# yuang-chen/of-spmm

Hardware: AMD Instinct MI355X
Metric: SpMM effective GFLOP/s + achieved HBM GB/s vs roofline, 1/2/4/8 MI355X (higher is better)
Workload: dtype f32; 1 GPU; products: CSR 2449029x2449029, 123718280 nnz x dense N=128; m=2449029, k=2449029, nnz=123718280, n=128, index=int32, parallelism=single GPU

## Files before the change

of-spmm_amd/csrc/ofx_internal.h:

```cpp
#ifndef OFX_INTERNAL_H_
#define OFX_INTERNAL_H_

#include <stdarg.h>
#include <stdint.h>
#include <stdio.h>

#include "ofx_spmm.h"

namespace ofx {
int fail(int code, const char* fmt, ...) __attribute__((format(printf, 2, 3)));
void clear_error();

int guard_exception(const char* fn);
template <typename F>
inline int guarded(const char* fn, F&& body) noexcept {
  try {
    return body();
  } catch (...) {
    return guard_exception(fn);
  }
}

unsigned* device_error_words();
int take_device_error(const char* where);
int64_t debug_knob(int knob, int64_t dflt);

const char* versioned_struct_problem(const void* p, uint32_t min_size);
int read_options(const ofx_spmm_options* in, ofx_spmm_options* out, const char* fn);
}

#define OFX_READ_OPTIONS(opts, fn)                                                 \
  ofx_spmm_options ofx_opts_copy_;                                                 \
  do {                                                                             \
    if (const int ofx_ro_ = ::ofx::read_options((opts), &ofx_opts_copy_, (fn))) return ofx_ro_; \
    (opts) = &ofx_opts_copy_;                                                      \
  } while (0)

#define OFX_TAKE_DEVICE_ERROR(where)                                    \
  do {                                                                  \
    if (const int ofx_de_ = ::ofx::take_device_error(where)) return ofx_de_; \
  } while (0)

#define OFX_HIP_CHECK(expr)                                                                 \
  do {                                                                                      \
    hipError_t ofx_e_ = (expr);                                                             \
    if (ofx_e_ != hipSuccess) {                                                             \
      (void)hipGetLastError();       \
      return ::ofx::fail(OFX_EDEVICE, "%s failed: %s (%s:%d)", #expr,                       \
                         hipGetErrorString(ofx_e_), __FILE__, __LINE__);                    \
    }                                                                                       \
  } while (0)

#define OFX_REQUIRE(cond, code, ...)              \
  do {                                            \
    if (!(cond)) return ::ofx::fail(code, __VA_ARGS__); \
  } while (0)

#endif
```

of-spmm_amd/csrc/spmm_common.h:

```cpp
#ifndef OFX_SPMM_COMMON_H_
#define OFX_SPMM_COMMON_H_

#include <stdint.h>
#include <string.h>

#include "ofx_spmm.h"

#if defined(__HIPCC__) || defined(__HIP__)
#include <hip/hip_runtime.h>
#define OFX_HD __host__ __device__ __forceinline__
#else
#define OFX_HD static inline
#endif

namespace ofx {

struct bf16 {
  uint16_t x;
};
struct f16 {
  uint16_t x;
};

OFX_HD float bits_to_f32(uint32_t u) { return __builtin_bit_cast(float, u); }
OFX_HD uint32_t f32_to_bits(float f) { return __builtin_bit_cast(uint32_t, f); }

OFX_HD float bf16_to_f32(uint16_t h) { return bits_to_f32(uint32_t(h) << 16); }
OFX_HD uint16_t f32_to_bf16(float f) {
#if defined(__HIP_DEVICE_COMPILE__)
  return __builtin_bit_cast(uint16_t, (__bf16)f);
#else
  const uint32_t u = f32_to_bits(f);
  if ((u & 0x7fffffffu) > 0x7f800000u) return uint16_t((u >> 16) | 0x40u);
  return uint16_t((u + 0x7fffu + ((u >> 16) & 1u)) >> 16);
#endif
}
OFX_HD float f16_to_f32(uint16_t h) { return float(__builtin_bit_cast(_Float16, h)); }
OFX_HD uint16_t f32_to_f16(float f) { return __builtin_bit_cast(uint16_t, _Float16(f)); }

OFX_HD float round_bf16(float f) {
#if defined(__HIP_DEVICE_COMPILE__)
  return (float)(__bf16)f;
#else
  const uint32_t u = f32_to_bits(f);
  if ((u & 0x7fffffffu) > 0x7f800000u) return bits_to_f32((u & 0xffff0000u) | 0x400000u);
  return bits_to_f32((u + 0x7fffu + ((u >> 16) & 1u)) & 0xffff0000u);
#endif
}

template <typename T>
struct Num;
template <>
struct Num<float> {
  using acc = float;
  OFX_HD static float load(float v) { return v; }
  OFX_HD static float store(float a) { return a; }
  OFX_HD static float mul(float v, float b) { return v * b; }
};
template <>
struct Num<double> {
  using acc = double;
  OFX_HD static double load(double v) { return v; }
  OFX_HD static double store(double a) { return a; }
  OFX_HD static double mul(double v, double b) { return v * b; }
};
template <>
struct Num<bf16> {
  using acc = float;
  OFX_HD static float load(bf16 v) { return bf16_to_f32(v.x); }
  OFX_HD static bf16 store(float a) { return bf16{f32_to_bf16(a)}; }
  OFX_HD static float mul(float v, float b) { return round_bf16(v * b); }
};
template <>
struct Num<f16> {
  using acc = float;
  OFX_HD static float load(f16 v) { return f16_to_f32(v.x); }
  OFX_HD static f16 store(float a) { return f16{f32_to_f16(a)}; }
  OFX_HD static float mul(float v, float b) { return float(_Float16(v * b)); }
};

template <typename T>
OFX_HD T epilogue(typename Num<T>::acc acc, const T* bias, int64_t c, int act) {
  T y = Num<T>::store(acc);
  if (bias) y = Num<T>::store(Num<T>::load(y) + Num<T>::load(bias[c]));
  if (act == OFX_ACT_RELU && Num<T>::load(y) <= typename Num<T>::acc(0))
    y = Num<T>::store(typename Num<T>::acc(0));
  return y;
}

template <typename T>
OFX_HD T poison_value() {
  return Num<T>::store(typename Num<T>::acc(__builtin_nan("")));
}

OFX_HD int dtype_size(int dt) {
  switch (dt) {
    case OFX_DT_FLOAT: return 4;
    case OFX_DT_DOUBLE: return 8;
    case OFX_DT_INT32: return 4;
    case OFX_DT_INT64: return 8;
    case OFX_DT_FLOAT16: return 2;
    case OFX_DT_BFLOAT16: return 2;
    default: return 0;
  }
}
OFX_HD bool is_index_dtype(int dt) { return dt == OFX_DT_INT32 || dt == OFX_DT_INT64; }
OFX_HD bool is_value_dtype(int dt) {
  return dt == OFX_DT_FLOAT || dt == OFX_DT_DOUBLE || dt == OFX_DT_FLOAT16 ||
         dt == OFX_DT_BFLOAT16;
}

OFX_HD int64_t default_split(int64_t n) {
  int64_t t = n > 0 ? (int64_t)65536 / n : 512;
  if (t < 128) t = 128;
  if (t > 512) t = 512;
  int64_t p = 128;
  while (p * 2 <= t) p *= 2;
  return p;
}

struct Schedule {
  int64_t split;
  int64_t chunk;
  int64_t heavy;
  int32_t variant;
  int32_t planned;
  int32_t force_bin;
};

static inline Schedule resolve_schedule(int64_t n, const ofx_spmm_options* o) {
  Schedule s;
  s.variant = o ? o->variant : 0;
  s.planned = o ? o->planned : 0;
  s.force_bin = 0;
  const int64_t h = o ? o->heavy_threshold : 0;
  s.heavy = h > 0 ? h : (h < 0 ? INT64_MAX : 0);
  if (o && o->ordered) {
    s.split = INT64_MAX;
    s.chunk = INT64_MAX;
    return s;
  }
  s.split = (o && o->split_threshold > 0) ? o->split_threshold : default_split(n);
  s.chunk = (o && o->chunk > 0) ? o->chunk : s.split;
  if (s.chunk > s.split) s.chunk = s.split;
  return s;
}

OFX_HD int64_t auto_heavy(int64_t nrows, int64_t nnz) {
  const int64_t mean = nrows > 0 ? (nnz + nrows - 1) / nrows : 1;
  return 5 * mean < 16 ? 16 : 5 * mean;
}

OFX_HD int64_t num_chunks(int64_t len, int64_t chunk) { return len / chunk; }

OFX_HD uint64_t splitmix64(uint64_t x) {
  x += 0x9e3779b97f4a7c15ull;
  x = (x ^ (x >> 30)) * 0xbf58476d1ce4e5b9ull;
  x = (x ^ (x >> 27)) * 0x94d049bb133111ebull;
  return x ^ (x >> 31);
}
OFX_HD uint64_t hash2(uint64_t seed, uint64_t i) { return splitmix64(splitmix64(seed) ^ i); }
OFX_HD float u_pm1(uint64_t h) { return float((int64_t)(h >> 40) - (1 << 23)) * (1.0f / (1 << 23)); }
OFX_HD float exact_val(uint64_t h) {
  const float t[4] = {-2.f, -1.f, 1.f, 2.f};
  return t[(h >> 33) & 3];
}
OFX_HD float exact_dense(uint64_t h) { return float((int)((h >> 33) % 17) - 8); }

}

#endif
```

of-spmm_amd/csrc/spmm_csr_impl.h:

```cpp
#ifndef OFX_SPMM_CSR_IMPL_H_
#define OFX_SPMM_CSR_IMPL_H_
#pragma clang fp contract(off)

#include <hip/hip_runtime.h>

#include <algorithm>
#include <climits>
#include <cstdio>
#include <cstring>
#include <type_traits>

#include "ofx_internal.h"
#include "spmm_common.h"
#include "spmm_plan.h"
#include "spmm_launch.h"
#include "dbg_bounds.h"

namespace ofx {
namespace {


using plan::WorkList;
using plan::WsLayout;
using plan::launch_plan;
// ... 741 lines not shown
          PA x[QR];
#pragma unroll
          for (int q = 0; q < QR; ++q)
            if (i + q < cnt) x[q] = *reinterpret_cast<const PA*>(buf + (i + q) * W + gl * VEC);
#pragma unroll
          for (int q = 0; q < QR; ++q)
            if (i + q < cnt)
#pragma unroll
              for (int e = 0; e < VEC; ++e) acc[e] = acc[e] + x[q].v[e];
        }
      }
    }
  };
  span_load(0, rc, rv);
  span_store(0, rc, rv);
  __syncthreads();
  span_load(1, rc, rv);
  static_assert(D == 4, "small form: the load ring below is written out for D = 4");
  P b0[UW], b1[UW], b2[UW], b3[UW];
  issue(0, b0);
  issue(1, b1);
  issue(2, b2);
  issue(3, b3);
  static_assert(S == 2 * D, "small form: a span is two turns of the ring");
  int64_t k0 = 0;
  for (; k0 + S <= nb; k0 += S) {
    step(k0 + 0, b0, false);
    step(k0 + 1, b1, false);
    step(k0 + 2, b2, false);
    step(k0 + 3, b3, false);
    step(k0 + 4, b0, true);
    step(k0 + 5, b1, false);
    step(k0 + 6, b2, false);
    step(k0 + 7, b3, false);
  }
  if (k0 + 0 < nb) step(k0 + 0, b0, false);
  if (k0 + 1 < nb) step(k0 + 1, b1, false);
  if (k0 + 2 < nb) step(k0 + 2, b2, false);
  if (k0 + 3 < nb) step(k0 + 3, b3, false);
  if (k0 + 4 < nb) step(k0 + 4, b0, false);
  if (k0 + 5 < nb) step(k0 + 5, b1, false);
  if (k0 + 6 < nb) step(k0 + 6, b2, false);
  if (kpc > 0) {
#pragma unroll
    for (int e = 0; e < VEC; ++e) acc[e] = total[e] + acc[e];
  }
  __syncthreads();
}

template <typename T, typename I, typename K>
__global__ void __launch_bounds__(64 * K::WPB)
    spmm_small_kernel(const I* __restrict__ rp, const I* __restrict__ col,
                      const T* __restrict__ val, const I* __restrict__ vperm,
                      const T* __restrict__ B, int64_t ldb, int64_t kb, T* __restrict__ C,
                      int64_t ldc, int64_t row_begin, int64_t nrows, int64_t n, int64_t split,
                      int64_t chunk,
                      int64_t light, const T* __restrict__ bias, int act) {
  using SF = SmallForm<T, I, K>;
  using A = typename Num<T>::acc;
  constexpr int VEC = K::VEC, LPR = K::LPR, W = SF::W, RPB = SF::RPB;
  __shared__ __attribute__((aligned(16))) SmallLds<T, I, K> lds;
  __shared__ int heavy_rows[RPB];
  __shared__ int nheavy;
  const int lane = threadIdx.x & 63;
  const int wave = threadIdx.x >> 6;
  const int gl = lane & (LPR - 1);
  const int gbase = lane & ~(LPR - 1);
  const int q = LPR == 64 ? 0 : lane / LPR;
  const int gb = wave * SF::G + q;
  const int64_t row0 = (int64_t)blockIdx.x * RPB;
  if (threadIdx.x == 0) nheavy = 0;
  __syncthreads();
  const int64_t lr = row0 + gb;
  if (lr < nrows) {
    const int64_t rs = (int64_t)OFX_LD(rp + (row_begin + lr));
    const int64_t re = (int64_t)OFX_LD(rp + (row_begin + lr + 1));
    const int64_t len = re - rs;
    if (len > light || len > split) {
      if (gl == 0) heavy_rows[atomicAdd(&nheavy, 1)] = gb;
    } else {
      for (int64_t c0 = 0; c0 < n; c0 += W) {
        const int64_t cc = c0 + (int64_t)gl * VEC;
        const bool active = cc < n;
        A acc[VEC];
#pragma unroll
        for (int e = 0; e < VEC; ++e) acc[e] = A(0);
        accumulate<T, I, K>(col, val, vperm, brows<T, K::BUF>(B, c0, cc, active, ldb, kb), rs, re, gl, gbase,
                            active, acc);
        if (active) store_row<T, VEC, K::NT>(C + lr * ldc + cc, acc, bias ? bias + cc : nullptr, act);
      }
    }
  }
  __syncthreads();
  const int nh = nheavy;
  const bool chain = wave == 0 && q == 0;
  for (int h = 0; h < nh; ++h) {
    const int64_t hr = row0 + heavy_rows[h];
    const int64_t rs = (int64_t)OFX_LD(rp + (row_begin + hr));
    const int64_t re = (int64_t)OFX_LD(rp + (row_begin + hr + 1));
    const bool split_row = re - rs > split;
    const int64_t nc = split_row ? num_chunks(re - rs, chunk) : 1;
    const bool one_pass = split_row && chunk % SF::NB == 0;
    for (int64_t c0 = 0; c0 < n; c0 += W) {
      const int64_t cc = c0 + (int64_t)gl * VEC;
      const bool active = cc < n;
      const BRows<T, K::BUF> br = brows<T, K::BUF>(B, c0, cc, active, ldb, kb);
      A total[VEC], acc[VEC];
#pragma unroll
      for (int e = 0; e < VEC; ++e) total[e] = A(0);
      if (one_pass) {
#pragma unroll
        for (int e = 0; e < VEC; ++e) acc[e] = A(0);
        block_accumulate<T, I, K>(col, val, vperm, br, rs, re, gb, gl, chain, lds, acc,
                                  chunk / SF::NB, nc);
        if (chain && active) store_row<T, VEC, K::NT>(C + hr * ldc + cc, acc, bias ? bias + cc : nullptr, act);
        continue;
      }
      for (int64_t ci = 0; ci < nc; ++ci) {
        int64_t j0 = rs, j1 = re;
        if (split_row) {
          j0 = rs + ci * chunk;
          j1 = (re - j0 - chunk < chunk) ? re : j0 + chunk;
        }
#pragma unroll
        for (int e = 0; e < VEC; ++e) acc[e] = A(0);
        block_accumulate<T, I, K>(col, val, vperm, br, j0, j1, gb, gl, chain, lds, acc);
        if (split_row) {
#pragma unroll
          for (int e = 0; e < VEC; ++e) total[e] = total[e] + acc[e];
        }
      }
      if (chain && active)
        store_row<T, VEC, K::NT>(C + hr * ldc + cc, split_row ? total : acc,
                                 bias ? bias + cc : nullptr, act);
    }
  }
}

#ifdef OFX_AB_WPE
#define OFX_MAIN_WPE __attribute__((amdgpu_waves_per_eu(OFX_AB_WPE)))
#else
#define OFX_MAIN_WPE
#endif
template <typename T>
__device__ __attribute__((noinline)) void poison_output(T* __restrict__ C, int64_t ldc,
                                                        int64_t nrows, int64_t n) {
  const T p = poison_value<T>();
  const int64_t total = nrows * n;
  const int64_t stride = (int64_t)gridDim.x * blockDim.x;
  for (int64_t e = (int64_t)blockIdx.x * blockDim.x + threadIdx.x; e < total; e += stride)
    C[(e / n) * ldc + e % n] = p;
}

template <typename T, typename I, typename K>
__global__ void __launch_bounds__(64 * K::WPB) OFX_MAIN_WPE
    spmm_main_kernel(const I* __restrict__ rp, const I* __restrict__ col,
                     const T* __restrict__ val, const I* __restrict__ vperm,
                     const T* __restrict__ B, int64_t ldb, int64_t kb,
                     T* __restrict__ C, int64_t ldc, int64_t row_begin, int64_t nrows, int64_t n,
                     int64_t split, int64_t chunk, int64_t heavy,
                     const unsigned long long* __restrict__ counters,
                     const int64_t* __restrict__ items, const int64_t* __restrict__ order,
                     typename Num<T>::acc* __restrict__ part, const T* __restrict__ bias,
                     int act, int64_t wave_blocks, int64_t block_base,
                     unsigned* __restrict__ arrive, unsigned* err) {
  using A = typename Num<T>::acc;
  constexpr int VEC = K::VEC, LPR = K::LPR, kWaves = K::WPB;
  const int64_t bid = block_base + (int64_t)blockIdx.x;
  if (counters != nullptr && !plan::plan_valid(counters)) {
    if (bid == 0 && threadIdx.x == 0) plan::raise_device_error(err, plan::kErrPlanInvalid);
    poison_output<T>(C, ldc, nrows, n);
    return;
  }
  constexpr int GPW = 64 / LPR;
  const int lane = threadIdx.x & 63;
  const int wave = __builtin_amdgcn_readfirstlane(threadIdx.x >> 6);
  const int gl = lane & (LPR - 1);
  const int gbase = lane & ~(LPR - 1);
  const int gsub = LPR == 64 ? 0 : lane / LPR;
  if constexpr (K::WH && LPR < 64) {
    using KW = WaveMap<K>;
    constexpr int WV = KW::VEC, WL = KW::LPR;
    if (bid < wave_blocks) {
      const int wgl = lane & (WL - 1);
      const int64_t nchunks = (int64_t)OFX_LD(counters + 0);
      const int64_t nheavy = (int64_t)OFX_LD(counters + 3) - (int64_t)OFX_LD(counters + 2);
      for (int64_t w = bid * kWaves + wave; w < nchunks + nheavy; w += wave_blocks * kWaves) {
        int64_t wr, wc = -1;
        if (w < nchunks) {
          wr = OFX_LD(items + (2 * w + 0));
          wc = OFX_LD(items + (2 * w + 1));
        } else {
          wr = plan::order_row(order, nrows, nheavy, w - nchunks);
        }
        wr = uniform64(wr);
        wc = uniform64(wc);
        const int64_t rs = (int64_t)OFX_LD(rp + (row_begin + wr));
        const int64_t re = (int64_t)OFX_LD(rp + (row_begin + wr + 1));
        int64_t j0 = rs, j1 = re;
        if (wc >= 0) {
          j0 = rs + wc * chunk;
          j1 = (re - j0 - chunk < chunk) ? re : j0 + chunk;
        }
        for (int64_t c0 = 0; c0 < n; c0 += (int64_t)WL * WV) {
          int64_t cc = c0 + (int64_t)wgl * WV;
          const bool active = cc < n;
          if constexpr (K::SH && WV > 1) {
            if (active && cc + WV > n) cc = n - WV;
          }
          A acc[WV];
#pragma unroll
          for (int e = 0; e < WV; ++e) acc[e] = A(0);
          if constexpr (K::XL) {
            __shared__ A xl_lds[K::WPB][KW::XL_FLOATS];
            accumulate_wave_xl<T, I, KW>(col, val, vperm, brows<T, K::BUF>(B, c0, cc, active, ldb, kb),
                                         j0, j1, lane, wgl, xl_lds[wave], acc);
          } else {
            accumulate_wave<T, I, KW>(col, val, vperm, brows<T, K::BUF>(B, c0, cc, active, ldb, kb),
                                      j0, j1, lane, wgl, acc);
          }
          if (active && lane < WL) {
            if (wc >= 0)
              store_partial<A, WV, K::LR>(part + w * n + cc, acc);
            else
              store_row<T, WV, K::NT>(C + wr * ldc + cc, acc, bias ? bias + cc : nullptr, act);
          }
        }
        if constexpr (K::LR) {
          if (wc >= 0)
            hub_tail<T, WV, WL, K::SH && (WV > 1)>(arrive, w - wc, num_chunks(re - rs, chunk), part, C, ldc,
                                       wr, n, wgl, lane < WL, 0, bias, act);
        }
      }
      return;
    }
  }
  if constexpr (K::BI) {
    if (bid < wave_blocks) {
      __shared__ __attribute__((aligned(16))) SmallLds<T, I, K> lds;
      constexpr int W = SmallForm<T, I, K>::W;
      const int64_t w = bid;
      const int64_t nchunks = (int64_t)OFX_LD(counters + 0);
      const int64_t nheavy = (int64_t)OFX_LD(counters + 3) - (int64_t)OFX_LD(counters + 2);
      if (w >= nchunks + nheavy) return;
      int64_t wr, wc = -1;
      if (w < nchunks) {
        wr = OFX_LD(items + (2 * w + 0));
        wc = OFX_LD(items + (2 * w + 1));
      } else {
        wr = plan::order_row(order, nrows, nheavy, w - nchunks);
      }
      wr = uniform64(wr);
      wc = uniform64(wc);
      const int64_t rs = (int64_t)OFX_LD(rp + (row_begin + wr));
      const int64_t re = (int64_t)OFX_LD(rp + (row_begin + wr + 1));
      int64_t j0 = rs, j1 = re;
      if (wc >= 0) {
        j0 = rs + wc * chunk;
        j1 = (re - j0 - chunk < chunk) ? re : j0 + chunk;
      }
      const int gb = wave * GPW + gsub;
      const bool chain = wave == 0 && gsub == 0;
      for (int64_t c0 = 0; c0 < n; c0 += W) {
        const int64_t cc = c0 + (int64_t)gl * VEC;
        const bool active = cc < n;
        A acc[VEC];
#pragma unroll
        for (int e = 0; e < VEC; ++e) acc[e] = A(0);
        block_accumulate<T, I, K>(col, val, vperm, brows<T, K::BUF>(B, c0, cc, active, ldb, kb), j0, j1, gb, gl,
                                  chain, lds, acc);
        if (chain && active) {
          if (wc >= 0)
            store_partial<A, VEC, K::LR>(part + w * n + cc, acc);
          else
            store_row<T, VEC, K::NT>(C + wr * ldc + cc, acc, bias ? bias + cc : nullptr, act);
        }
      }
      if constexpr (K::LR) {
        if (wc >= 0 && chain)
          hub_tail<T, VEC, LPR, K::SH>(arrive, w - wc, num_chunks(re - rs, chunk), part, C, ldc, wr,
                                       n, gl, true, gbase, bias, act);
      }
      return;
    }
  }
  int64_t g = ((bid - ((K::WH || K::BI) ? wave_blocks : 0)) * kWaves + wave) * GPW +
              gsub;
  if constexpr ((K::WH && LPR < 64) || K::BI) {
    if (order != nullptr)
      g += (int64_t)OFX_LD(counters + 0) + (int64_t)OFX_LD(counters + 3) -
           (int64_t)OFX_LD(counters + 2);
  }
  constexpr int64_t kIdxExcluded = 16;
#if defined(OFX_LIGHT_ORDER)
  constexpr bool kIdx = false;
#else
  constexpr bool kIdx = true;
#endif
  int64_t lr, c = -1;
  bool by_index = false;
  if (order == nullptr) {
    if (g >= nrows) return;
    lr = g;
  } else {
    const int64_t nchunks = (int64_t)OFX_LD(counters + 0);
    const int64_t nhubs = (int64_t)OFX_LD(counters + 1);
    const int64_t nheavy = (int64_t)OFX_LD(counters + 3) - (int64_t)OFX_LD(counters + 2);
#if defined(OFX_LIGHT_INDEX)
    const bool idx = true;
#else
    const bool idx = kIdx && (nhubs + nheavy) * kIdxExcluded <= nrows;
#endif
    if (g < nchunks) {
      lr = OFX_LD(items + (2 * g + 0));
      c = OFX_LD(items + (2 * g + 1));
    } else if (g < nchunks + nheavy || !idx) {
      const int64_t q = g - nchunks;
      if (q >= nrows - nhubs) return;
      lr = plan::order_row(order, nrows, nheavy, q);
    } else {
      lr = g - nchunks - nheavy;
      if (lr >= nrows) return;
      by_index = true;
    }
  }
  if constexpr (LPR == 64) {
    lr = uniform64(lr);
    c = uniform64(c);
  }
  const int64_t rs = (int64_t)OFX_LD(rp + (row_begin + lr));
  const int64_t re = (int64_t)OFX_LD(rp + (row_begin + lr + 1));
  if (by_index && (re - rs > split || re - rs > heavy)) return;
  int64_t j0 = rs, j1 = re;
  if (c >= 0) {
    j0 = rs + c * chunk;
    j1 = (re - j0 - chunk < chunk) ? re : j0 + chunk;
  }
  for (int64_t c0 = 0; c0 < n; c0 += (int64_t)LPR * VEC) {
    int64_t cc = c0 + (int64_t)gl * VEC;
    const bool active = cc < n;
    if constexpr (K::SH) {
      if (active && cc + VEC > n) cc = n - VEC;
    }
    A acc[VEC];
#pragma unroll
    for (int e = 0; e < VEC; ++e) acc[e] = A(0);
    accumulate<T, I, K>(col, val, vperm, brows<T, K::BUF>(B, c0, cc, active, ldb, kb), j0, j1, gl, gbase, active,
                        acc);
    if (active) {
      if (c >= 0)
        store_partial<A, VEC, K::LR>(part + g * n + cc, acc);
      else
        store_row<T, VEC, K::NT>(C + lr * ldc + cc, acc, bias ? bias + cc : nullptr, act);
    }
  }
  if constexpr (K::LR) {
    if (c >= 0)
      hub_tail<T, VEC, LPR, K::SH>(arrive, g - c, num_chunks(re - rs, chunk), part, C, ldc, lr, n,
                                   gl, true, gbase, bias, act);
  }
}


template <typename T, int VEC, int L>
__global__ void __launch_bounds__(kBlock)
    spmm_reduce_kernel(const unsigned long long* __restrict__ counters,
                       const int64_t* __restrict__ hubs,
                       const typename Num<T>::acc* __restrict__ part, T* __restrict__ C,
                       int64_t ldc, int64_t n, const T* __restrict__ bias, int act) {
#pragma clang fp contract(off)
  using A = typename Num<T>::acc;
  using P = Pack<A, VEC>;
  constexpr int kPre = 16;
  if (!plan::plan_valid(counters)) return;
  const int64_t nhubs = (int64_t)OFX_LD(counters + 1);
  const int gl = threadIdx.x % L;
  const int64_t groups = (int64_t)gridDim.x * (kBlock / L);
  for (int64_t h = (int64_t)blockIdx.x * (kBlock / L) + threadIdx.x / L; h < nhubs; h += groups) {
    const int64_t lr = OFX_LD(hubs + (3 * h + 0));
    const int64_t slot = OFX_LD(hubs + (3 * h + 1));
    const int64_t nc = OFX_LD(hubs + (3 * h + 2));
    for (int64_t c = (int64_t)gl * VEC; c < n; c += (int64_t)L * VEC) {
      const A* p = part + slot * n + c;
      A acc[VEC];
#pragma unroll
      for (int e = 0; e < VEC; ++e) acc[e] = A(0);
      int64_t q = 0;
      for (; q + kPre <= nc; q += kPre) {
        P v[kPre];
#pragma unroll
        for (int u = 0; u < kPre; ++u) v[u] = OFX_LD(reinterpret_cast<const P*>(p + (q + u) * n));
#pragma unroll
        for (int u = 0; u < kPre; ++u) {
#pragma unroll
          for (int e = 0; e < VEC; ++e) acc[e] = acc[e] + v[u].v[e];
        }
      }
      for (; q < nc; ++q) {
        const P v = OFX_LD(reinterpret_cast<const P*>(p + q * n));
#pragma unroll
        for (int e = 0; e < VEC; ++e) acc[e] = acc[e] + v.v[e];
      }
      if (bias && !OFX_DOK(bias + c, sizeof(T) * VEC)) continue;
#pragma unroll
      for (int e = 0; e < VEC; ++e) OFX_ST(&C[lr * ldc + c + e], epilogue<T>(acc[e], bias, c + e, act));
    }
  }
}

template <typename T, int VEC>
int launch_reduce_vec(hipStream_t s, int64_t max_hubs, int64_t n,
                      const unsigned long long* counters, const int64_t* hubs,
                      const typename Num<T>::acc* part, T* C, int64_t ldc, const T* bias, int act) {
  const int64_t lanes = (n + VEC - 1) / VEC;
  int l = 4;
  while (l < 64 && l < lanes) l *= 2;
  const int64_t per_block = kBlock / l;
  int64_t grid = (max_hubs + per_block - 1) / per_block;
  if (grid > kMaxReduceBlocks) grid = kMaxReduceBlocks;
#define OFX_REDUCE(LL)                                                                        \
  hipLaunchKernelGGL((spmm_reduce_kernel<T, VEC, LL>), dim3((unsigned)grid), dim3(kBlock), 0, s, \
                     counters, hubs, part, C, ldc, n, bias, act)
  switch (l) {
    case 4: OFX_REDUCE(4); break;
    case 8: OFX_REDUCE(8); break;
    case 16: OFX_REDUCE(16); break;
    case 32: OFX_REDUCE(32); break;
    default: OFX_REDUCE(64); break;
  }
#undef OFX_REDUCE
  OFX_HIP_CHECK(hipGetLastError());
  return OFX_OK;
}

template <typename T>
int launch_reduce(hipStream_t s, int64_t max_hubs, int64_t n, const unsigned long long* counters,
                  const int64_t* hubs, const typename Num<T>::acc* part, T* C, int64_t ldc,
                  const T* bias, int act) {
  using A = typename Num<T>::acc;
  constexpr int kVec = 16 / (int)sizeof(A);
  if ((n * (int64_t)sizeof(A)) % 16 == 0)
    return launch_reduce_vec<T, kVec>(s, max_hubs, n, counters, hubs, part, C, ldc, bias, act);
  return launch_reduce_vec<T, 1>(s, max_hubs, n, counters, hubs, part, C, ldc, bias, act);
}

int pick_vec(int elem_bytes, const Launch& L, int forced_vec, int cap = 16) {
  const int maxvec = std::min(16 / elem_bytes, cap);
  for (int v = maxvec; v >= 1; v /= 2) {
    if (forced_vec && v != forced_vec) continue;
    const size_t vb = (size_t)v * elem_bytes;
    if (L.n % v == 0 && L.ldb % v == 0 && L.ldc % v == 0 &&
        ((uintptr_t)L.b % vb) == 0 && ((uintptr_t)L.c % vb) == 0)
      return v;
  }
  return 0;
}

int pick_lpr(int64_t n, int vec) {
  const int64_t lanes = (n + vec - 1) / vec;
  int l = 4;
  while (l < 64 && l < lanes) l *= 2;
  return l;
}

template <typename T, typename I, typename K>
int describe_cfg(const Launch& L, const char* kind) {
  const char* form = std::strcmp(kind, "small") == 0 ? "small"
                     : K::BI                         ? "mid"
                     : (K::WH && K::HL > 0)          ? "narrow"
                     : K::PF                         ? "prefetch"
                                                     : "bandwidth";
  const size_t ws = std::strcmp(kind, "small") == 0
                        ? 0
                        : ws_layout(L.nrows, L.nnz, L.n, sizeof(typename Num<T>::acc), L.sched).total;
  std::snprintf(L.describe, L.describe_bytes,
                "form=%s kernel=%s VEC=%d LPR=%d U=%d WPB=%d NT=%d PF=%d WH=%d BI=%d BUF=%d SH=%d "
                "HL=%d HU=%d HV=%d XL=%d LR=%d elem=%d idx=%d ws=%zu",
                form, kind, K::VEC, K::LPR, K::U, K::WPB, (int)K::NT, (int)K::PF, (int)K::WH,
                (int)K::BI, (int)K::BUF, (int)K::SH, K::HL, K::HU, K::HV, (int)K::XL, (int)K::LR,
                (int)sizeof(T),
                (int)sizeof(I), ws);
  return OFX_OK;
}

#ifdef OFX_DEBUG_BOUNDS
template <typename T, typename I, typename K>
int debug_publish(const Launch& L, unsigned long long kind) {
  dbg::HostBounds hb;
  const int64_t si = (int64_t)sizeof(I), st = (int64_t)sizeof(T);
  hb.add(L.rp, (uint64_t)((L.row_begin + L.nrows + 1) * si));
  hb.add(L.col, (uint64_t)(L.nnz * si));
  hb.add(L.val, (uint64_t)(L.nnz * st));
  hb.add(L.vperm, (uint64_t)(L.nnz * si));
  if (L.b_rows > 0) hb.add(L.b, (uint64_t)(((L.b_rows - 1) * L.ldb + L.n) * st));
  hb.add(L.c, (uint64_t)(((L.nrows - 1) * L.ldc + L.n) * st));
  hb.add(L.ws, L.ws_bytes);
  hb.add(L.bias, (uint64_t)(L.n * st));
  void* zero = nullptr;
  OFX_HIP_CHECK(hipGetSymbolAddress(&zero, HIP_SYMBOL(g_zero_row)));
  hb.add(zero, kZeroRowBytes);
  const unsigned long long flags = (unsigned long long)K::NT | (unsigned long long)K::PF << 1 |
                                   (unsigned long long)K::BNT << 2 | (unsigned long long)K::WH << 3 |
                                   (unsigned long long)K::BI << 4 | (unsigned long long)K::BUF << 5 |
                                   (unsigned long long)K::SH << 6 | (unsigned long long)K::LR << 7;
  const unsigned long long tag = (unsigned long long)K::VEC | (unsigned long long)K::LPR << 8 |
                                 (unsigned long long)K::U << 16 | flags << 24 |
                                 (unsigned long long)K::HL << 32 | (unsigned long long)K::HU << 40 |
                                 kind << 48;
  OFX_REQUIRE(hb.publish(L.stream, tag) == 0, OFX_EDEVICE, "spmm_csr: debug bounds not published");
  return OFX_OK;
}
#endif

template <typename T, typename I, typename K>
int launch_cfg(const Launch& L) {
  if (L.describe != nullptr) return describe_cfg<T, I, K>(L, "main");
  using A = typename Num<T>::acc;
  constexpr int GPW = 64 / K::LPR;
  constexpr int64_t GPB = (int64_t)K::WPB * GPW;
  const I* rp = static_cast<const I*>(L.rp);
  const I* col = static_cast<const I*>(L.col);
  const T* val = static_cast<const T*>(L.val);
  const T* B = static_cast<const T*>(L.b);
  T* C = static_cast<T*>(L.c);
  const WsLayout w = ws_layout(L.nrows, L.nnz, L.n, sizeof(A), L.sched);
  const bool plan = w.total > 0;
#ifdef OFX_DEBUG_BOUNDS
  if (const int rc = debug_publish<T, I, K>(L, 1)) return rc;
#endif
  WorkList wl{};
  if (plan) {
    OFX_REQUIRE(L.ws != nullptr && L.ws_bytes >= w.total, OFX_EWORKSPACE,
                "spmm_csr: workspace of %zu bytes is smaller than the %zu bytes required",
                L.ws_bytes, w.total);
    if (L.sched.planned) {
      plan::worklist_of(w, static_cast<char*>(L.ws), &wl);
    } else {
      const int rc = launch_plan<I>(L.stream, rp, L.row_begin, L.nrows, L.nnz_est, L.sched, w,
                                    static_cast<char*>(L.ws), &wl);
      if (rc) return rc;
    }
  }
  unsigned long long* counters = wl.counters;
  int64_t *hub = wl.hubs, *items = wl.items, *order = wl.order;
  A* part = reinterpret_cast<A*>(wl.part);
  const int64_t heavy = L.sched.heavy == 0 ? auto_heavy(L.nrows, L.nnz_est) : L.sched.heavy;
  const int64_t heavy_bound =
      heavy == INT64_MAX ? 0 : std::min<int64_t>(L.nrows, L.nnz / (heavy + 1) + 1);
  const int64_t bi_items = w.max_chunks + heavy_bound;
  constexpr int64_t kWaveItemBlocks = 2048;
  const bool wh = K::WH && K::LPR < 64 && plan;
  const int64_t wave_blocks = wh ? std::min<int64_t>((bi_items + K::WPB - 1) / K::WPB, kWaveItemBlocks)
                              : (K::BI && plan) ? bi_items
                                                : 0;
  const int64_t work = L.nrows + (plan && !wh && !K::BI ? bi_items : 0);
  const int64_t grid = wave_blocks + (work + GPB - 1) / GPB;
  constexpr int64_t kLaunchBlocks = ((int64_t)1 << 31) / (64 * K::WPB);
  for (int64_t b0 = 0; b0 < grid; b0 += kLaunchBlocks) {
    const int64_t nb = std::min(kLaunchBlocks, grid - b0);
    hipLaunchKernelGGL((spmm_main_kernel<T, I, K>), dim3((unsigned)nb), dim3(64 * K::WPB), 0,
                       L.stream, rp, col, val, static_cast<const I*>(L.vperm), B, L.ldb, L.b_rows,
                       C, L.ldc, L.row_begin, L.nrows, L.n, plan ? L.sched.split : INT64_MAX,
                       plan ? L.sched.chunk : INT64_MAX, heavy, counters, items, order, part,
                       static_cast<const T*>(L.bias), L.act, wave_blocks, b0, wl.arrive,
                       plan ? device_error_words() : nullptr);
    OFX_HIP_CHECK(hipGetLastError());
  }
  if (plan && w.max_hubs > 0 && !K::LR)
    return launch_reduce<T>(L.stream, w.max_hubs, L.n, counters, hub, part, C, L.ldc,
                            static_cast<const T*>(L.bias), L.act);
  return OFX_OK;
}


template <typename T, typename I, typename K>
int launch_small(const Launch& L) {
  if (L.describe != nullptr) return describe_cfg<T, I, K>(L, "small");
  using SF = SmallForm<T, I, K>;
  const int64_t light =
      (L.sched.heavy > 0 && L.sched.heavy != INT64_MAX) ? L.sched.heavy : (int64_t)kSmallLight * K::U;
  const int64_t grid = (L.nrows + SF::RPB - 1) / SF::RPB;
#ifdef OFX_DEBUG_BOUNDS
  if (const int rc = debug_publish<T, I, K>(L, 2)) return rc;
#endif
  OFX_REQUIRE(grid < (int64_t)UINT32_MAX, OFX_EINVAL, "spmm_csr: too many rows (%lld)",
              (long long)L.nrows);
  hipLaunchKernelGGL((spmm_small_kernel<T, I, K>), dim3((unsigned)grid), dim3(64 * K::WPB), 0,
                     L.stream, static_cast<const I*>(L.rp), static_cast<const I*>(L.col),
                     static_cast<const T*>(L.val), static_cast<const I*>(L.vperm),
                     static_cast<const T*>(L.b), L.ldb, L.b_rows, static_cast<T*>(L.c), L.ldc,
                     L.row_begin,
                     L.nrows, L.n, L.sched.split, L.sched.chunk, light,
                     static_cast<const T*>(L.bias), L.act);
  OFX_HIP_CHECK(hipGetLastError());
  return OFX_OK;
}

template <typename T, typename I, typename K>
int launch_small_or_planned(const Launch& L) {
  if (use_small_form(L.nrows, L.nnz_est, L.n, L.sched)) return launch_small<T, I, K>(L);
  return launch_cfg<T, I, K>(L);
}

constexpr int64_t kNtBytes = int64_t(1) << 30;

template <typename T, typename I, int VEC>
int launch_vec_small(const Launch& L, int lpr) {
  constexpr int U = VEC * sizeof(T) <= 4 ? 32 : 16;
  switch (lpr) {
    case 4: return launch_small_or_planned<T, I, Cfg<VEC, 4, U, 4, false, true, false, true>>(L);
    case 8: return launch_small_or_planned<T, I, Cfg<VEC, 8, U, 4, false, true, false, true>>(L);
    case 16: return launch_small_or_planned<T, I, Cfg<VEC, 16, U, 4, false, true, false, true>>(L);
    case 32: return launch_small_or_planned<T, I, Cfg<VEC, 32, U, 4, false, true, false, true>>(L);
    case 64: return launch_small_or_planned<T, I, Cfg<VEC, 64, U, 4, false, false, false, false>>(L);
    default: return fail(OFX_EINVAL, "spmm_csr: unsupported lanes-per-row %d", lpr);
  }
}

template <typename T, typename I, int VEC, bool WH>
int launch_vec_pf(const Launch& L, int lpr) {
  constexpr int U = VEC * sizeof(T) <= 4 ? 32 : 16;
  switch (lpr) {
    case 4: return launch_cfg<T, I, Cfg<VEC, 4, U, 4, false, true, false, WH, false, true, 0, 16, false, kLR>>(L);
    case 8: return launch_cfg<T, I, Cfg<VEC, 8, U, 4, false, true, false, WH, false, true, 0, 16, false, kLR>>(L);
    case 16: return launch_cfg<T, I, Cfg<VEC, 16, U, 4, false, true, false, WH, false, true, 0, 16, false, kLR>>(L);
    case 32: return launch_cfg<T, I, Cfg<VEC, 32, U, 4, false, true, false, WH, false, true, 0, 16, false, kLR>>(L);
    case 64: return launch_cfg<T, I, Cfg<VEC, 64, U, 4, false, false, false, false, false, true, 0, 16, false, kLR>>(L);
    default: return fail(OFX_EINVAL, "spmm_csr: unsupported lanes-per-row %d", lpr);
  }
}

template <typename T, typename I, int VEC, bool SR>
int launch_vec_mid(const Launch& L, int lpr) {
  constexpr int U = SR ? (VEC * sizeof(T) <= 4 ? 32 : 16) : (VEC == 1 && sizeof(T) == 4 ? 16 : 8);
  switch (lpr) {
    case 4: return launch_cfg<T, I, Cfg<VEC, 4, U, 4, false, SR, false, false, true, true, 0, 16, false, kLR>>(L);
    case 8: return launch_cfg<T, I, Cfg<VEC, 8, U, 4, false, SR, false, false, true, true, 0, 16, false, kLR>>(L);
    case 16: return launch_cfg<T, I, Cfg<VEC, 16, U, 4, false, SR, false, false, true, true, 0, 16, false, kLR>>(L);
    case 32: return launch_cfg<T, I, Cfg<VEC, 32, U, 4, false, SR, false, false, true, true, 0, 16, false, kLR>>(L);
    case 64: return launch_cfg<T, I, Cfg<VEC, 64, U, 4, false, SR, false, false, true, true, 0, 16, false, kLR>>(L);
    default: return fail(OFX_EINVAL, "spmm_csr: unsupported lanes-per-row %d", lpr);
  }
}

template <typename T>
bool buffer_rows_ok(const Launch& L) {
  return (unsigned __int128)(L.b_rows + 1) * (unsigned __int128)L.ldb * sizeof(T) <
         ((unsigned __int128)1 << 32);
}

template <typename T, typename I, int VEC>
int launch_vec_global(const Launch& L, int lpr, bool nt) {
  switch (lpr) {
    case 4: return launch_cfg<T, I, Cfg<VEC, 4, 8, 4, false, false, false, false, false, false>>(L);
    case 8: return launch_cfg<T, I, Cfg<VEC, 8, 8, 4, false, false, false, false, false, false>>(L);
    case 16:
      if constexpr (VEC == 1 && sizeof(T) == 4)
        return launch_cfg<T, I, Cfg<1, 16, 16, 4, false, false, false, false, false, false>>(L);
      return launch_cfg<T, I, Cfg<VEC, 16, 8, 4, false, false, false, false, false, false>>(L);
    case 32:
      return nt ? launch_cfg<T, I, Cfg<VEC, 32, 8, 4, true, false, false, false, false, false>>(L)
                : launch_cfg<T, I, Cfg<VEC, 32, 8, 4, false, false, false, false, false, false>>(L);
    case 64:
      return nt ? launch_cfg<T, I, Cfg<VEC, 64, 8, 4, true, false, false, false, false, false>>(L)
                : launch_cfg<T, I, Cfg<VEC, 64, 8, 4, false, false, false, false, false, false>>(L);
    default: return fail(OFX_EINVAL, "spmm_csr: unsupported lanes-per-row %d", lpr);
  }
}

template <typename T, typename I, int VEC>
int launch_vec(const Launch& L, int lpr, bool nt) {
  const int v = L.sched.variant;
  if (!buffer_rows_ok<T>(L)) {
    OFX_REQUIRE(v == 0 || v == kForceBigVariant || v == kForceGlobalVariant || (v > 0 && v < 10000),
                OFX_EINVAL,
                "spmm_csr: variant %d needs B under 4 GiB (k=%lld, ldb=%lld)", v,
                (long long)L.b_rows, (long long)L.ldb);
    return launch_vec_global<T, I, VEC>(L, lpr, nt);
  }
  if (v == kForceSmallVariant || (v == 0 && use_small_form(L.nrows, L.nnz_est, L.n, L.sched)))
    return launch_vec_small<T, I, VEC>(L, lpr);
  if (v == kForceMidSmallVariant) return launch_vec_mid<T, I, VEC, true>(L, lpr);
  if (v == kForceMidVariant) return launch_vec_mid<T, I, VEC, false>(L, lpr);
  if (v == kForceWaveVariant) return launch_vec_pf<T, I, VEC, true>(L, lpr);
  if (v == kForcePrefetchVariant) return launch_vec_pf<T, I, VEC, false>(L, lpr);
  if (v == kForceGlobalVariant) return launch_vec_global<T, I, VEC>(L, lpr, nt);
  if (v == 0 && use_mid_form(L.nrows, L.nnz_est, L.n, L.sched)) {
// ... 178 lines not shown
```

of-spmm_amd/csrc/spmm_launch.h:

```cpp
#ifndef OFX_SPMM_LAUNCH_H_
#define OFX_SPMM_LAUNCH_H_

#include <hip/hip_runtime.h>

#include "spmm_common.h"

namespace ofx {

struct Launch {
  hipStream_t stream;
  const void *rp, *col, *val, *b;
  void* c;
  int64_t ldb, ldc, row_begin, nrows, n, nnz;
  Schedule sched;
  void* ws;
  size_t ws_bytes;
  const void* bias;
  int act;
  int64_t b_rows;
  const void* vperm;
  int64_t nnz_est;
  char* describe = nullptr;
  size_t describe_bytes = 0;
};

inline int64_t launch_nnz(int64_t m, int64_t nrows, int64_t nnz, const ofx_spmm_options* o) {
  if (m <= 0 || nrows >= m) return nnz;
  if (o != nullptr && o->range_nnz > 0) return o->range_nnz < nnz ? o->range_nnz : nnz;
  return (int64_t)((__int128)nnz * nrows / m);
}

constexpr int64_t kSmallRows = 32768;
constexpr int64_t kSmallFormNnz = int64_t(1) << 17;
constexpr int64_t kSmallFormElems = int64_t(1) << 23;
constexpr int kSmallLight = 2;
constexpr int kForceSmallVariant = 30000;

inline bool use_small_form(int64_t nrows, int64_t nnz, int64_t n, const Schedule& s) {
  if (s.variant == kForceSmallVariant) return true;
  return s.variant == 0 && nrows <= kSmallRows && nnz <= kSmallFormNnz &&
         nnz <= kSmallFormElems / (n > 0 ? n : 1);
}

constexpr int64_t kMidFormElems = int64_t(1) << 28;
constexpr int64_t kBlockItemMin = 64;
constexpr int kForceMidVariant = 30001;
constexpr int kForceMidSmallVariant = 30002;

inline bool use_mid_form(int64_t nrows, int64_t nnz, int64_t n, const Schedule& s) {
  if (s.variant == kForceMidVariant || s.variant == kForceMidSmallVariant) return true;
  return s.variant == 0 && nrows <= kSmallRows && !use_small_form(nrows, nnz, n, s) &&
         nnz <= kMidFormElems / (n > 0 ? n : 1);
}

constexpr int64_t kPrefetchNnz = int64_t(3) << 20;

inline bool use_prefetch_form(int64_t nrows, int64_t nnz, int64_t n, const Schedule& s) {
  return s.variant == 0 && !use_small_form(nrows, nnz, n, s) && !use_mid_form(nrows, nnz, n, s) &&
         nnz <= kPrefetchNnz;
}

constexpr int kForceBigVariant = 30003;
constexpr int kForceWaveVariant = 30004;
constexpr int kForcePrefetchVariant = 30005;
constexpr int kForceGlobalVariant = 30006;

inline bool is_form_variant(int v) {
  return v == kForceSmallVariant || v == kForceMidVariant || v == kForceMidSmallVariant ||
         v == kForceBigVariant || v == kForceWaveVariant || v == kForcePrefetchVariant ||
         v == kForceGlobalVariant;
}

inline Schedule launch_schedule(int64_t nrows, int64_t nnz, int64_t n, Schedule s) {
  if (!use_mid_form(nrows, nnz, n, s)) return s;
  s.force_bin = 1;
  if (s.heavy == 0) {
    const int64_t h = auto_heavy(nrows, nnz);
    s.heavy = h > kBlockItemMin ? h : kBlockItemMin;
  }
  return s;
}

template <typename T, typename I>
int launch_typed(const Launch& L);
template <typename T, typename I>
int launch_tuned(const Launch& L, int id);

}

#endif
```

Measured before the change: 3727 GFLOP/s.

## Overlap planned heavy-row work on an auxiliary stream with direct light-row kernel

Adds a per-device auxiliary stream with fork/join events. For large matrices with low mean row length, the planner, the heavy/split-item main kernel and the hub reduction run on the aux stream, while a separate main-kernel instantiation handles rows directly on the caller's stream, with no dependency on the plan. A finish kernel then poisons the output if the plan was invalid. The aim is to hide the planning and heavy-row latency behind the bulk row work. The cost is extra launches, event synchronisation, a mutex, and contention between the two kernels for CUs and bandwidth.

```diff
diff --git a/of-spmm_amd/csrc/aux_stream.cpp b/of-spmm_amd/csrc/aux_stream.cpp
--- /dev/null
+++ b/of-spmm_amd/csrc/aux_stream.cpp
@@ -0,0 +1,50 @@
+#include <hip/hip_runtime.h>
+
+#include <mutex>
+
+#include "ofx_internal.h"
+
+namespace ofx {
+namespace {
+constexpr int kMaxDevices = 64;
+struct Slot {
+  std::once_flag once;
+  AuxStream aux;
+  bool ok = false;
+};
+Slot g_slots[kMaxDevices];
+
+void create(Slot* s) {
+  hipStream_t st = nullptr;
+  hipEvent_t fork = nullptr, lead = nullptr, join = nullptr;
+  hipError_t e = hipStreamCreateWithFlags(&st, hipStreamNonBlocking);
+  if (e == hipSuccess) e = hipEventCreateWithFlags(&fork, hipEventDisableTiming);
+  if (e == hipSuccess) e = hipEventCreateWithFlags(&lead, hipEventDisableTiming);
+  if (e == hipSuccess) e = hipEventCreateWithFlags(&join, hipEventDisableTiming);
+  if (e != hipSuccess) {
+    (void)hipGetLastError();
+    if (join) (void)hipEventDestroy(join);
+    if (lead) (void)hipEventDestroy(lead);
+    if (fork) (void)hipEventDestroy(fork);
+    if (st) (void)hipStreamDestroy(st);
+    return;
+  }
+  s->aux.stream = st;
+  s->aux.fork = fork;
+  s->aux.lead = lead;
+  s->aux.join = join;
+  s->ok = true;
+}
+}
+
+AuxStream* aux_stream_current_device() {
+  int dev = -1;
+  if (hipGetDevice(&dev) != hipSuccess || dev < 0 || dev >= kMaxDevices) {
+    (void)hipGetLastError();
+    return nullptr;
+  }
+  Slot* s = &g_slots[dev];
+  std::call_once(s->once, create, s);
+  return s->ok ? &s->aux : nullptr;
+}
+}
diff --git a/of-spmm_amd/csrc/ofx_internal.h b/of-spmm_amd/csrc/ofx_internal.h
--- a/of-spmm_amd/csrc/ofx_internal.h
+++ b/of-spmm_amd/csrc/ofx_internal.h
@@ -4,6 +4,8 @@
 #include <stdarg.h>
 #include <stdint.h>
 #include <stdio.h>
+
+#include <mutex>
 
 #include "ofx_spmm.h"
 
@@ -24,6 +26,15 @@
 unsigned* device_error_words();
 int take_device_error(const char* where);
 int64_t debug_knob(int knob, int64_t dflt);
+
+struct AuxStream {
+  void* stream = nullptr;
+  void* fork = nullptr;
+  void* lead = nullptr;
+  void* join = nullptr;
+  std::mutex mu;
+};
+AuxStream* aux_stream_current_device();
 
 const char* versioned_struct_problem(const void* p, uint32_t min_size);
 int read_options(const ofx_spmm_options* in, ofx_spmm_options* out, const char* fn);
diff --git a/of-spmm_amd/csrc/spmm_common.h b/of-spmm_amd/csrc/spmm_common.h
--- a/of-spmm_amd/csrc/spmm_common.h
+++ b/of-spmm_amd/csrc/spmm_common.h
@@ -126,6 +126,7 @@
   int32_t variant;
   int32_t planned;
   int32_t force_bin;
+  int32_t overlap;
 };
 
 static inline Schedule resolve_schedule(int64_t n, const ofx_spmm_options* o) {
@@ -133,6 +134,7 @@
   s.variant = o ? o->variant : 0;
   s.planned = o ? o->planned : 0;
   s.force_bin = 0;
+  s.overlap = 0;
   const int64_t h = o ? o->heavy_threshold : 0;
   s.heavy = h > 0 ? h : (h < 0 ? INT64_MAX : 0);
   if (o && o->ordered) {
diff --git a/of-spmm_amd/csrc/spmm_csr_impl.h b/of-spmm_amd/csrc/spmm_csr_impl.h
--- a/of-spmm_amd/csrc/spmm_csr_impl.h
+++ b/of-spmm_amd/csrc/spmm_csr_impl.h
@@ -917,7 +917,9 @@
     C[(e / n) * ldc + e % n] = p;
 }
 
-template <typename T, typename I, typename K>
+constexpr int kMainAll = 0, kMainRows = 1, kMainItems = 2;
+
+template <typename T, typename I, typename K, int MODE = kMainAll>
 __global__ void __launch_bounds__(64 * K::WPB) OFX_MAIN_WPE
     spmm_main_kernel(const I* __restrict__ rp, const I* __restrict__ col,
                      const T* __restrict__ val, const I* __restrict__ vperm,
@@ -932,11 +934,17 @@
   using A = typename Num<T>::acc;
   constexpr int VEC = K::VEC, LPR = K::LPR, kWaves = K::WPB;
   const int64_t bid = block_base + (int64_t)blockIdx.x;
-  if (counters != nullptr && !plan::plan_valid(counters)) {
-    if (bid == 0 && threadIdx.x == 0) plan::raise_device_error(err, plan::kErrPlanInvalid);
-    poison_output<T>(C, ldc, nrows, n);
-    return;
-  }
+  if constexpr (MODE == kMainItems) {
+    if (!plan::plan_valid(counters)) return;
+  } else if constexpr (MODE == kMainAll) {
+    if (counters != nullptr && !plan::plan_valid(counters)) {
+      if (bid == 0 && threadIdx.x == 0) plan::raise_device_error(err, plan::kErrPlanInvalid);
+      poison_output<T>(C, ldc, nrows, n);
+      return;
+    }
+  }
+  static_assert(MODE == kMainAll || !((K::WH && K::LPR < 64) || K::BI || K::LR),
+                "the overlapped schedule serves the bandwidth form only");
   constexpr int GPW = 64 / LPR;
   const int lane = threadIdx.x & 63;
   const int wave = __builtin_amdgcn_readfirstlane(threadIdx.x >> 6);
@@ -1064,7 +1072,21 @@
 #endif
   int64_t lr, c = -1;
   bool by_index = false;
-  if (order == nullptr) {
+  if constexpr (MODE == kMainRows) {
+    if (g >= nrows) return;
+    lr = g;
+    by_index = true;
+  } else if constexpr (MODE == kMainItems) {
+    const int64_t nchunks = (int64_t)OFX_LD(counters + 0);
+    const int64_t nheavy = (int64_t)OFX_LD(counters + 3) - (int64_t)OFX_LD(counters + 2);
+    if (g < nchunks) {
+      lr = OFX_LD(items + (2 * g + 0));
+      c = OFX_LD(items + (2 * g + 1));
+    } else {
+      if (g >= nchunks + nheavy) return;
+      lr = plan::order_row(order, nrows, nheavy, g - nchunks);
+    }
+  } else if (order == nullptr) {
     if (g >= nrows) return;
     lr = g;
   } else {
@@ -1126,6 +1148,17 @@
   }
 }
 
+constexpr int kFinishBlocks = 256;
+
+template <typename T>
+__global__ void __launch_bounds__(kBlock)
+    spmm_finish_kernel(const unsigned long long* __restrict__ counters, T* __restrict__ C,
+                       int64_t ldc, int64_t nrows, int64_t n, unsigned* err) {
+  if (plan::plan_valid(counters)) return;
+  if (blockIdx.x == 0 && threadIdx.x == 0) plan::raise_device_error(err, plan::kErrPlanInvalid);
+  poison_output<T>(C, ldc, nrows, n);
+}
+
 
 template <typename T, int VEC, int L>
 __global__ void __launch_bounds__(kBlock)
@@ -1228,6 +1261,9 @@
   return l;
 }
 
+template <typename K>
+constexpr bool kOverlapCfg = !K::PF && !K::WH && !K::BI && !K::LR && K::BUF;
+
 template <typename T, typename I, typename K>
 int describe_cfg(const Launch& L, const char* kind) {
   const char* form = std::strcmp(kind, "small") == 0 ? "small"
@@ -1240,11 +1276,12 @@
                         : ws_layout(L.nrows, L.nnz, L.n, sizeof(typename Num<T>::acc), L.sched).total;
   std::snprintf(L.describe, L.describe_bytes,
                 "form=%s kernel=%s VEC=%d LPR=%d U=%d WPB=%d NT=%d PF=%d WH=%d BI=%d BUF=%d SH=%d "
-                "HL=%d HU=%d HV=%d XL=%d LR=%d elem=%d idx=%d ws=%zu",
+                "HL=%d HU=%d HV=%d XL=%d LR=%d elem=%d idx=%d ws=%zu overlap=%d",
                 form, kind, K::VEC, K::LPR, K::U, K::WPB, (int)K::NT, (int)K::PF, (int)K::WH,
                 (int)K::BI, (int)K::BUF, (int)K::SH, K::HL, K::HU, K::HV, (int)K::XL, (int)K::LR,
                 (int)sizeof(T),
-                (int)sizeof(I), ws);
+                (int)sizeof(I), ws,
+                (int)(kOverlapCfg<K> && ws > 0 && use_overlap(L.nrows, L.nnz_est, L.sched)));
   return OFX_OK;
 }
 
@@ -1277,6 +1314,74 @@
 }
 #endif
 
+inline bool stream_capturing(hipStream_t s) {
+  hipStreamCaptureStatus st = hipStreamCaptureStatusNone;
+  if (hipStreamIsCapturing(s, &st) != hipSuccess) {
+    (void)hipGetLastError();
+    return true;
+  }
+  return st != hipStreamCaptureStatusNone;
+}
+
+template <typename T, typename I, typename K>
+int launch_overlapped(const Launch& L, const WsLayout& w, AuxStream* ax) {
+  using A = typename Num<T>::acc;
+  constexpr int GPW = 64 / K::LPR;
+  constexpr int64_t GPB = (int64_t)K::WPB * GPW;
+  constexpr int64_t kLaunchBlocks = ((int64_t)1 << 31) / (64 * K::WPB);
+  const I* rp = static_cast<const I*>(L.rp);
+  const I* col = static_cast<const I*>(L.col);
+  const T* val = static_cast<const T*>(L.val);
+  const I* vperm = static_cast<const I*>(L.vperm);
+  const T* B = static_cast<const T*>(L.b);
+  const T* bias = static_cast<const T*>(L.bias);
+  T* C = static_cast<T*>(L.c);
+  hipStream_t s = L.stream, a = static_cast<hipStream_t>(ax->stream);
+  hipEvent_t fork = static_cast<hipEvent_t>(ax->fork), join = static_cast<hipEvent_t>(ax->join);
+  hipEvent_t lead = static_cast<hipEvent_t>(ax->lead);
+  const int64_t heavy = L.sched.heavy == 0 ? auto_heavy(L.nrows, L.nnz_est) : L.sched.heavy;
+  const int64_t heavy_bound =
+      heavy == INT64_MAX ? 0 : std::min<int64_t>(L.nrows, L.nnz / (heavy + 1) + 1);
+  unsigned* err = device_error_words();
+  WorkList wl{};
+  plan::worklist_of(w, static_cast<char*>(L.ws), &wl);
+  A* part = reinterpret_cast<A*>(wl.part);
+  auto launch_main = [&](auto mode, hipStream_t st, int64_t groups) -> int {
+    const int64_t grid = (groups + GPB - 1) / GPB;
+    for (int64_t b0 = 0; b0 < grid; b0 += kLaunchBlocks) {
+      const int64_t nb = std::min(kLaunchBlocks, grid - b0);
+      hipLaunchKernelGGL((spmm_main_kernel<T, I, K, decltype(mode)::value>), dim3((unsigned)nb),
+                         dim3(64 * K::WPB), 0, st, rp, col, val, vperm, B, L.ldb, L.b_rows, C,
+                         L.ldc, L.row_begin, L.nrows, L.n, L.sched.split, L.sched.chunk, heavy,
+                         wl.counters, wl.items, wl.order, part, bias, L.act, (int64_t)0, b0,
+                         wl.arrive, err);
+      OFX_HIP_CHECK(hipGetLastError());
+    }
+    return OFX_OK;
+  };
+  std::lock_guard<std::mutex> lock(ax->mu);
+  OFX_HIP_CHECK(hipEventRecord(fork, s));
+  OFX_HIP_CHECK(hipStreamWaitEvent(a, fork, 0));
+  OFX_HIP_CHECK(hipEventRecord(lead, a));
+  int rc = OFX_OK;
+  if (!L.sched.planned)
+    rc = launch_plan<I>(a, rp, L.row_begin, L.nrows, L.nnz_est, L.sched, w,
+                        static_cast<char*>(L.ws), &wl);
+  if (rc == OFX_OK)
+    rc = launch_main(std::integral_constant<int, kMainItems>{}, a, w.max_chunks + heavy_bound);
+  if (rc == OFX_OK && w.max_hubs > 0)
+    rc = launch_reduce<T>(a, w.max_hubs, L.n, wl.counters, wl.hubs, part, C, L.ldc, bias, L.act);
+  OFX_HIP_CHECK(hipEventRecord(join, a));
+  OFX_HIP_CHECK(hipStreamWaitEvent(s, lead, 0));
+  if (rc == OFX_OK) rc = launch_main(std::integral_constant<int, kMainRows>{}, s, L.nrows);
+  OFX_HIP_CHECK(hipStreamWaitEvent(s, join, 0));
+  if (rc != OFX_OK) return rc;
+  hipLaunchKernelGGL((spmm_finish_kernel<T>), dim3(kFinishBlocks), dim3(kBlock), 0, s,
+                     wl.counters, C, L.ldc, L.nrows, L.n, err);
+  OFX_HIP_CHECK(hipGetLastError());
+  return OFX_OK;
+}
+
 template <typename T, typename I, typename K>
 int launch_cfg(const Launch& L) {
   if (L.describe != nullptr) return describe_cfg<T, I, K>(L, "main");
@@ -1298,6 +1403,13 @@
     OFX_REQUIRE(L.ws != nullptr && L.ws_bytes >= w.total, OFX_EWORKSPACE,
                 "spmm_csr: workspace of %zu bytes is smaller than the %zu bytes required",
                 L.ws_bytes, w.total);
+#ifndef OFX_DEBUG_BOUNDS
+    if constexpr (kOverlapCfg<K>) {
+      if (use_overlap(L.nrows, L.nnz_est, L.sched) && !stream_capturing(L.stream)) {
+        if (AuxStream* ax = aux_stream_current_device()) return launch_overlapped<T, I, K>(L, w, ax);
+      }
+    }
+#endif
     if (L.sched.planned) {
       plan::worklist_of(w, static_cast<char*>(L.ws), &wl);
     } else {
diff --git a/of-spmm_amd/csrc/spmm_launch.h b/of-spmm_amd/csrc/spmm_launch.h
--- a/of-spmm_amd/csrc/spmm_launch.h
+++ b/of-spmm_amd/csrc/spmm_launch.h
@@ -65,6 +65,17 @@
 constexpr int kForcePrefetchVariant = 30005;
 constexpr int kForceGlobalVariant = 30006;
 
+constexpr int64_t kOverlapMeanDiv = 8;
+constexpr int64_t kOverlapMinNnz = int64_t(1) << 26;
+constexpr int kForceOverlapVariant = 30007;
+constexpr int kForceSerialVariant = 30008;
+
+inline bool use_overlap(int64_t nrows, int64_t nnz, const Schedule& s) {
+  if (s.overlap != 0) return s.overlap > 0;
+  if (s.variant != 0 || s.split == INT64_MAX || nrows <= 0) return false;
+  return nnz >= kOverlapMinNnz && (__int128)nnz * kOverlapMeanDiv <= (__int128)s.split * nrows;
+}
+
 inline bool is_form_variant(int v) {
   return v == kForceSmallVariant || v == kForceMidVariant || v == kForceMidSmallVariant ||
          v == kForceBigVariant || v == kForceWaveVariant || v == kForcePrefetchVariant ||
@@ -72,6 +83,13 @@
 }
 
 inline Schedule launch_schedule(int64_t nrows, int64_t nnz, int64_t n, Schedule s) {
+  if (s.variant == kForceOverlapVariant) {
+    s.variant = kForceBigVariant;
+    s.overlap = 1;
+  } else if (s.variant == kForceSerialVariant) {
+    s.variant = 0;
+    s.overlap = -1;
+  }
   if (!use_mid_form(nrows, nnz, n, s)) return s;
   s.force_bin = 1;
   if (s.heavy == 0) {
```

Result: no change. 3739 GFLOP/s, median of 4 (+0.3%).
